# simzero/cudaParticlesFoam

Hardware: AMD Instinct MI355X
Metric: Mparticle-steps/s (higher is better)
Workload: dtype f64

## Files before the change

cudaparticlesfoam_amd/csrc/cpf_stream.hip:

```cpp
#include "cpf_stream_ops.h"

#include <hip/hip_ext.h>

#include <type_traits>

namespace cpf {

#ifndef CPF_STREAM_SLOTS
#define CPF_STREAM_SLOTS 6
#endif
#ifndef CPF_STREAM_SLOTS_FIXED
#define CPF_STREAM_SLOTS_FIXED 9
#endif
#ifndef CPF_STREAM_WAVES
#define CPF_STREAM_WAVES 7
#endif
constexpr int kSlotStride = 8;
#ifndef CPF_STREAM_GATHER_LANES
#define CPF_STREAM_GATHER_LANES 32
#endif
constexpr int kStreamGatherLanes = CPF_STREAM_GATHER_LANES;
#ifndef CPF_STREAM_PAIRED
#define CPF_STREAM_PAIRED 0
#endif
#ifndef CPF_STREAM_INROUND
#define CPF_STREAM_INROUND 0
#endif
#ifndef CPF_STREAM_HIT_POOL
#define CPF_STREAM_HIT_POOL 40
#endif
constexpr int kVertexTets = 12;
#ifndef CPF_VERTEX_BLOCKS
#define CPF_VERTEX_BLOCKS 4
#endif
#ifndef CPF_VERTEX_PICK_UNROLL
#define CPF_VERTEX_PICK_UNROLL 12
#endif
constexpr int kVertexBlocks = CPF_VERTEX_BLOCKS;
constexpr int kStreamSparsePerCell = 8;
constexpr int kSitOut = INT32_MIN + 7;

struct StreamKernArgs {
    double *x, *y, *z; int32_t* cell; const int64_t* gid; double* vel; int64_t n; double dt, sigma; uint32_t step0; int nCyc;
    uint32_t seed; MeshView m; unsigned long long* counters; StreamArgs sa;
};
static_assert(offsetof(StreamKernArgs, x) == 0 && offsetof(StreamKernArgs, cell) == 24, "kernarg_cloud_ptrs reads bytes 0..31");
constexpr int kKernArgHitSpill = (int)(offsetof(StreamKernArgs, sa) + offsetof(StreamArgs, hitSpill));
constexpr int kKernArgZBad = (int)(offsetof(StreamKernArgs, sa) + offsetof(StreamArgs, zBad));
constexpr int kKernArgGid = (int)offsetof(StreamKernArgs, gid), kKernArgSigma = (int)offsetof(StreamKernArgs, sigma);
constexpr int kKernArgStep0 = (int)offsetof(StreamKernArgs, step0), kKernArgSeed = (int)offsetof(StreamKernArgs, seed);
#ifndef CPF_STREAM_BROWN_KERNARG
#define CPF_STREAM_BROWN_KERNARG 1
#endif

#ifndef CPF_STREAM_L1_ZERO_SKIP
#define CPF_STREAM_L1_ZERO_SKIP 1
#endif
#ifndef CPF_STREAM_LAZY_USED
#define CPF_STREAM_LAZY_USED 1
#endif
#ifndef CPF_STREAM_BOX_SPARSE
#define CPF_STREAM_BOX_SPARSE 1
#endif
#ifndef CPF_STREAM_FLAT_KICK
#define CPF_STREAM_FLAT_KICK 0
#endif
#ifndef CPF_STREAM_FLAT_ZERO_SKIP
#define CPF_STREAM_FLAT_ZERO_SKIP 0
#endif
#ifndef CPF_STREAM_FLAT_Z
#define CPF_STREAM_FLAT_Z 1
#endif
#ifndef CPF_STREAM_SLOTS_BOX
#define CPF_STREAM_SLOTS_BOX 9
#endif
#ifndef CPF_STREAM_SLOTS_BOX_B
#define CPF_STREAM_SLOTS_BOX_B 12
#endif
#ifndef CPF_STREAM_WAVES_BOX_B
#define CPF_STREAM_WAVES_BOX_B 6
#endif
#ifndef CPF_STREAM_WAVES_BOX
#define CPF_STREAM_WAVES_BOX 6
#endif
#ifndef CPF_STREAM_WAVES_B1
#define CPF_STREAM_WAVES_B1 5
#endif
#ifndef CPF_STREAM_WAVES_L2
#define CPF_STREAM_WAVES_L2 6
#endif
#ifndef CPF_STREAM_WAVES_B0
#define CPF_STREAM_WAVES_B0 7
#endif
#ifndef CPF_STREAM_HIT_POOL_B0
#define CPF_STREAM_HIT_POOL_B0 18
#endif
#ifndef CPF_STREAM_WAVES_FLAT
#define CPF_STREAM_WAVES_FLAT CPF_STREAM_WAVES
#endif
#ifndef CPF_STREAM_WAVES_FLAT_BODY
#define CPF_STREAM_WAVES_FLAT_BODY 0
#endif
#ifndef CPF_FLAT_ROUND_GATHER
#define CPF_FLAT_ROUND_GATHER 1
#endif
#ifndef CPF_FLAT_ROUND_HINTS
#define CPF_FLAT_ROUND_HINTS 1
#endif
#ifndef CPF_FLAT_ROUND_ONE_HOOK
#define CPF_FLAT_ROUND_ONE_HOOK 1
#endif
#ifndef CPF_FLAT_ROUND_MASK
#define CPF_FLAT_ROUND_MASK 1
#endif
#ifndef CPF_FLAT_ROUND_OUTCOME
#define CPF_FLAT_ROUND_OUTCOME 1
#endif
#ifndef CPF_STREAM_SLOTS_BROWN
#define CPF_STREAM_SLOTS_BROWN 10
#endif
#ifndef CPF_STREAM_HIT_REGS_L2
#define CPF_STREAM_HIT_REGS_L2 0
#endif
#ifndef CPF_STREAM_WAVES_VERTEX
#define CPF_STREAM_WAVES_VERTEX 4
#endif
template <bool BROWNIAN, bool STORE_VEL, bool STATS, int LOOKUP>
struct StreamShape {
    static constexpr LookupMode mode = lookup_traits(LOOKUP);
    static_assert(mode.id == LOOKUP, "LOOKUP: a mode of kLookupModes");
    static constexpr int slots = [] {
        if (!mode.fixed) return CPF_STREAM_SLOTS;
        if (mode.box) return BROWNIAN ? CPF_STREAM_SLOTS_BOX_B : CPF_STREAM_SLOTS_BOX;
        if (BROWNIAN && LOOKUP == kLookupFixed) return CPF_STREAM_SLOTS_BROWN;
        return CPF_STREAM_SLOTS_FIXED;
    }();
    static_assert(slots >= 4 && slots <= 32, "slots");
    static constexpr int stride = mode.box ? 4 : kSlotStride;
    static constexpr bool hitInRegs = !BROWNIAN && (!mode.bigCells || CPF_STREAM_HIT_REGS_L2);
    static constexpr int pool = [] {
        if (hitInRegs) return 1;
        if (mode.mixed) return 16;
        if (BROWNIAN && LOOKUP == kLookupLoop) return CPF_STREAM_HIT_POOL_B0;
        return CPF_STREAM_HIT_POOL;
    }();
    static constexpr int waves = [] {
        if (STORE_VEL || STATS) return 1;
        if (mode.gatherAhead != 0) return BROWNIAN ? 4 : 5;
        if (BROWNIAN && mode.mixed) return 5;
        if (BROWNIAN && mode.box) return CPF_STREAM_WAVES_BOX_B;
        if (BROWNIAN) return LOOKUP == kLookupFixed ? CPF_STREAM_WAVES_B1 : CPF_STREAM_WAVES_B0;
        if (mode.bigCells) return CPF_STREAM_WAVES_L2;
        if (mode.box) return CPF_STREAM_WAVES_BOX;
        if (mode.mixed) return 6;
        if (LOOKUP == kLookupFlatLoop) return CPF_STREAM_WAVES_FLAT;
        return CPF_STREAM_WAVES;
    }();
};
#if CPF_STREAM_SLOTS == 6 && CPF_STREAM_SLOTS_FIXED == 9 && CPF_STREAM_SLOTS_BROWN == 10 && CPF_STREAM_SLOTS_BOX == 9 && CPF_STREAM_SLOTS_BOX_B == 12 && \
    CPF_STREAM_WAVES == 7 && CPF_STREAM_WAVES_B0 == 7 && CPF_STREAM_WAVES_B1 == 5 && CPF_STREAM_WAVES_L2 == 6 && CPF_STREAM_WAVES_BOX == 6 && \
    CPF_STREAM_WAVES_BOX_B == 6 && CPF_STREAM_WAVES_FLAT == 7 && CPF_STREAM_HIT_POOL == 40 && CPF_STREAM_HIT_POOL_B0 == 18 && CPF_STREAM_HIT_REGS_L2 == 0
template <int LOOKUP>
constexpr bool shape_is(int slots, int waves, int pool, int slotsB, int wavesB, int poolB) {
    using P = StreamShape<false, false, false, LOOKUP>; using B = StreamShape<true, false, false, LOOKUP>;
    return P::slots == slots && P::waves == waves && P::pool == pool && B::slots == slotsB && B::waves == wavesB && B::pool == poolB;
}
static_assert(shape_is<0>(6, 7, 1, 6, 7, 18) && shape_is<1>(9, 7, 1, 10, 5, 40) && shape_is<2>(9, 6, 16, 9, 5, 16) && shape_is<3>(9, 6, 1, 9, 5, 16) &&
              shape_is<4>(9, 5, 1, 9, 4, 40) && shape_is<5>(6, 6, 1, 6, 5, 16) && shape_is<6>(9, 6, 1, 12, 6, 40) && shape_is<8>(6, 7, 1, 6, 7, 40) &&
              shape_is<9>(9, 7, 1, 9, 7, 40) && shape_is<11>(9, 6, 1, 12, 5, 16), "StreamShape: slots, waves, pool per mode");
#endif

template <bool BROWNIAN, bool REFLECT, bool STORE_VEL, bool STATS, int LOOKUP, bool VERTEX, bool ZSET = false>
__device__ __forceinline__ void stream_body(
    const int64_t* __restrict__ gid, double* __restrict__ vel, int64_t n, double dt, double sigma, uint32_t step0,
    int nCyc, uint32_t seed, const MeshView& m, unsigned long long* __restrict__ counters, const StreamArgs& sa, const VertexField& vf) {
    using Shape = StreamShape<BROWNIAN, STORE_VEL, STATS, LOOKUP>;
    constexpr bool LOOKUP_FIXED = Shape::mode.fixed, mixed = Shape::mode.mixed, bigCells = Shape::mode.bigCells, BOX = Shape::mode.box;
    constexpr bool FLAT = Shape::mode.flat, HIT_IN_REGS = Shape::hitInRegs;
    constexpr int kGatherAhead = Shape::mode.gatherAhead, NS = Shape::slots, kStride = Shape::stride, kPool = Shape::pool;
    constexpr unsigned kRecBytes = 32u * kStride;
    constexpr unsigned ALL = NS == 32 ? 0xFFFFFFFFu : ((1u << NS) - 1u);
    __shared__ double4 slots[NS][kStride];
    __shared__ unsigned sCnt[4];
    constexpr bool kInRound = CPF_STREAM_INROUND == 2 || (CPF_STREAM_INROUND == 1 && BROWNIAN);
    static_assert(!(kInRound && mixed), "in-round reflection knows neither face groups nor two-record cells");
    static_assert(!ZSET || (FLAT && !BROWNIAN && !VERTEX), "settled z: the flat walk without the kick or the vertex advect");
    __shared__ double sLane[ZSET ? 2 : 3][64];
    __shared__ double sPool[3][kPool];
    __shared__ unsigned sPoolUsed;
    __shared__ double sPre[ZSET ? 160 : (BROWNIAN ? 288 : 224)];
    __shared__ double sCone[VERTEX ? kVertexBlocks : 1][VERTEX ? kVertexTets * 10 : 1];
    double(*sE)[64] = sLane;
    const int lane = threadIdx.x;
    const unsigned ul = threadIdx.x;
    const unsigned preBase = uniform32(lds_addr(sPre));
    const unsigned slotBase = uniform32(lds_addr(slots));
    const int tpc = sa.tilesPerChunk;
    constexpr bool kMaskBusy = ZSET && CPF_FLAT_ROUND_MASK != 0, kPlainOutcome = ZSET && CPF_FLAT_ROUND_OUTCOME != 0;
    constexpr bool kFlatGather = ZSET && CPF_FLAT_ROUND_GATHER != 0, kHints = ZSET && CPF_FLAT_ROUND_HINTS != 0;
    constexpr bool kOneHook = ZSET && CPF_FLAT_ROUND_ONE_HOOK != 0;
    const bool zKeep = ZSET || (FLAT && CPF_STREAM_FLAT_Z != 0 && sa.zSettled != 0);
    auto park = [&](const D3& e) __attribute__((always_inline)) {
        sE[0][lane] = e.x; sE[1][lane] = e.y;
        if (!ZSET) sE[2][lane] = e.z;
    };
    auto parked = [&]() __attribute__((always_inline)) -> D3 {
        if (ZSET) return {sE[0][lane], sE[1][lane], 0.0};
        return {sE[0][lane], sE[1][lane], sE[2][lane]};
    };
    const bool zFold = !BOX && BROWNIAN && REFLECT && m.zThin != 0;
    const bool zLast = !FLAT && !BROWNIAN && m.zPairLast != 0;
    const bool flatKick = zFold && m.zSide0 != 0;
    const unsigned nTiles = (unsigned)((n + 63) >> 6);
    const unsigned nFull = (unsigned)(n >> 6), nTail = (unsigned)n & 63u;
    const unsigned big = sa.bigChunks;
    const unsigned nChunks = big + (nTiles - big * (unsigned)tpc);
    auto chunk_first = [&](unsigned c) -> unsigned {
        return c < big ? c * (unsigned)tpc : big * (unsigned)tpc + (c - big);
    };
    auto chunk_tiles = [&](unsigned c, unsigned firstTile) -> int {
        if (c >= nChunks) return 0;
        const unsigned k = nTiles - firstTile;
        const unsigned want = c < big ? (unsigned)tpc : 1u;
        return (int)(k < want ? k : want);
    };
    auto chunk_of = [&](unsigned j) -> unsigned {
        const unsigned long long c = (unsigned long long)(blockIdx.x & (kStreamGroups - 1)) + (unsigned long long)kStreamGroups * j;
        return c < (unsigned long long)nChunks ? (unsigned)c : nChunks;
    };
    StepStats st = {0, 0, 0, 0};
#ifdef CPF_STREAM_TIMELINE
    const uint64_t tl0 = __builtin_amdgcn_s_memrealtime();
    unsigned tlTiles = 0, tlRounds = 0;
    unsigned tlWaitRec = 0, tlWaitEnd = 0, tlMissRounds = 0;
    unsigned long long* const tlH = (!STORE_VEL && vel != nullptr && (sa.debug & 4)) ? reinterpret_cast<unsigned long long*>(vel) + 8 * 16384 : nullptr;
    unsigned tlVis = 0, tlRoundIdx = 0;
#endif

    for (unsigned k = blockIdx.x; k < (unsigned)kStreamGroups; k += gridDim.x)
        if (lane == 0) sa.grabNext[k * kStreamCounterStride] = 0u;
    const unsigned grp = blockIdx.x & (kStreamGroups - 1);
    unsigned* const myGrab = sa.grab + grp * kStreamCounterStride;

    auto prefetch = [&](unsigned t, const CloudPtrs& cp) __attribute__((always_inline)) -> int {
        double* const x = cp.x; double* const y = cp.y; double* const z = cp.z; int32_t* const cell = cp.cell;
        t = uniform32(t);
        const int64_t b = (int64_t)t * 64;
        unsigned ul = threadIdx.x;
        asm volatile("" : "+v"(ul));
        if (t < nFull) {
            const char* s1 = (ul < 32u ? reinterpret_cast<const char*>(x + b) : reinterpret_cast<const char*>(y + b)) + (ul & 31u) * 16u;
            glds16(s1, preBase);
            if (zKeep) {
                if (ul < 16u) glds16(reinterpret_cast<const char*>(cell + b) + ul * 16u, preBase + 1024u);
            } else if (ul < 48u) {
                const char* s2 = ul < 32u ? reinterpret_cast<const char*>(z + b) + ul * 16u
                                          : reinterpret_cast<const char*>(cell + b) + (ul - 32u) * 16u;
                glds16(s2, preBase + 1024u);
            }
            if (BROWNIAN) {
                const int64_t* const g = CPF_STREAM_BROWN_KERNARG ? static_cast<const int64_t*>(kernarg_pointer<kKernArgGid>()) : gid;
                if (g != nullptr) {
                    if (ul < 32u) glds16(reinterpret_cast<const char*>(g + b) + ul * 16u, preBase + 1792u);
                    return 3;
                }
            }
            return 2;
        }
        const unsigned lim = nTail - 1u;
        const unsigned l = ul < lim ? ul : lim;
        if (zKeep) {
            const double vx = (x + b)[l], vy = (y + b)[l];
            const int vc = (cell + b)[l];
            sPre[ul] = vx; sPre[64 + ul] = vy;
            reinterpret_cast<int*>(sPre + 128)[ul] = vc;
        } else {
        const double vx = (x + b)[l], vy = (y + b)[l], vz = (z + b)[l];
        const int vc = (cell + b)[l];
        sPre[ul] = vx; sPre[64 + ul] = vy; sPre[128 + ul] = vz;
        reinterpret_cast<int*>(sPre + 192)[ul] = vc;
        }
        if (BROWNIAN) {
            const int64_t* const g = CPF_STREAM_BROWN_KERNARG ? static_cast<const int64_t*>(kernarg_pointer<kKernArgGid>()) : gid;
            if (g != nullptr) reinterpret_cast<int64_t*>(sPre + 224)[ul] = (g + b)[l];
        }
        return 0;
    };

    unsigned got0 = 0;
    if (lane == 0) got0 = grab_sync(myGrab);
    const unsigned chunk0 = chunk_of(uniform32(got0));
    if (chunk_tiles(chunk0, chunk_first(chunk0)) > 0) {
        int tagv = -1;
        unsigned fifo = 0;

        unsigned tile = chunk_first(chunk0);
        int tilesLeft = chunk_tiles(chunk0, tile);
        (void)prefetch(tile, kernarg_cloud_ptrs());
        wait_vmcnt<0>();

        bool havePrev = false;
        unsigned rtile = 0;
        double rvx = 0, rvy = 0, rvz = 0;
        bool ralive = false;
        int rc = 0;
        unsigned rlim = 63;

        for (;;) {
            tile = uniform32(tile);
            const unsigned plim = tile < nFull ? 63u : nTail - 1u;
            double px = sPre[ul], py = sPre[64 + ul], pz = 0.0;
            int pc;
            if (zKeep) pc = reinterpret_cast<const int*>(sPre + 128)[ul];
            else { pz = sPre[128 + ul]; pc = reinterpret_cast<const int*>(sPre + 192)[ul]; }
            uint64_t pid = 0;
            if (BROWNIAN) {
                const bool haveIds = (CPF_STREAM_BROWN_KERNARG ? kernarg_pointer<kKernArgGid>() : (void*)gid) != nullptr;
                pid = haveIds ? (uint64_t) reinterpret_cast<const int64_t*>(sPre + 224)[ul] : (uint64_t)tile * 64 + ul;
            }
            if (ul > plim || pc < 0) pc = CPF_CELL_FROZEN;
            if (FLAT && !ZSET && !zKeep && ballot64(pc >= 0 && !(fabs(pz) <= 1.7976931348623157e308)) != 0ull) {
                unsigned* const bad = static_cast<unsigned*>(kernarg_pointer<kKernArgZBad>());
                if (bad != nullptr && lane == 0) *bad = 1u;
            }

            int cur = pc;
            int key2 = 0, carNext = 0, carBest = -1;
            double carDT = 2.0;
            D3 S_ = {px, py, pz}, v = {0, 0, 0};
            const uint64_t id = pid;

            unsigned ntile = 0;
            int ntilesLeft = 0;

            auto hook = [&](const D3& prev) __attribute__((always_inline)) -> int {
                int younger = 0;
                __builtin_amdgcn_sched_barrier(0);
                if (tilesLeft > 1) {
                    ntile = tile + 1;
                    ntilesLeft = tilesLeft - 1;
                } else {
                    unsigned got = 0;
                    if (lane == 0) got = grab_sync(myGrab);
                    const unsigned nxt = chunk_of(uniform32(got));
                    ntile = chunk_first(nxt);
                    ntilesLeft = chunk_tiles(nxt, ntile);
                }
                const CloudPtrs cp = kernarg_cloud_ptrs();
                double* const x = cp.x; double* const y = cp.y; double* const z = cp.z; int32_t* const cell = cp.cell;
                if (havePrev && !(sa.debug & 1)) {
                    const int64_t b = (int64_t)uniform32(rtile) * 64;
                    if (STORE_VEL && ralive) {
                        double* vv = vel + 3 * b;
                        async_store(vv, ul * 24u, rvx); async_store(vv + 1, ul * 24u, rvy); async_store(vv + 2, ul * 24u, rvz);
                    }
                    if (ul <= rlim) {
                        async_store(x + b, ul * 8u, prev.x); async_store(y + b, ul * 8u, prev.y);
                        if (!zKeep) async_store(z + b, ul * 8u, prev.z);
                        async_store(cell + b, ul * 4u, rc);
                    }
                    younger += zKeep ? 3 : 4;
                }
                if (ntilesLeft > 0 && !(sa.debug & 2)) younger += prefetch(ntile, cp);
                __builtin_amdgcn_sched_barrier(0);
                return younger;
            };

            bool busy = false;
            unsigned long long busyM = 0ull;
            bool zUnclear = false;
            int token = INT32_MIN, h = 0, j = 0;
            int hitAt = -1;
            D3 hitReg = {0, 0, 0};
            auto park_hit = [&](const D3& Hp) __attribute__((always_inline)) {
                if (HIT_IN_REGS) { hitReg = Hp; return; }
                if (hitAt < 0) hitAt = (int)atomicAdd(&sPoolUsed, 1u);
                if (hitAt < kPool) { sPool[0][hitAt] = Hp.x; sPool[1][hitAt] = Hp.y; sPool[2][hitAt] = Hp.z; }
                else {
                    double* sp = static_cast<double*>(kernarg_pointer<kKernArgHitSpill>()) + (size_t)blockIdx.x * kStreamHitSpillDoubles;
                    async_store(sp, ul * 8u, Hp.x); async_store(sp + 64, ul * 8u, Hp.y); async_store(sp + 128, ul * 8u, Hp.z);
                }
            };

            auto cycle_begin = [&](int c) __attribute__((always_inline)) {
                if (cur < 0) cur = CPF_CELL_FROZEN;
                busy = cur >= 0;
                if (kMaskBusy) busyM = ballot64(cur >= 0);
                token = INT32_MIN; h = 0; j = 0;
                if (bigCells) key2 = 0;
                if (!HIT_IN_REGS && REFLECT) { hitAt = -1; if (lane == 0) sPoolUsed = 0u; }
                zUnclear = false;
                if (STATS && busy) ++st.steps;
                if (VERTEX) {
                    bool slow = busy;
#if defined(CPF_VERTEX_AB) && CPF_VERTEX_AB == 1
                    if (busy) { const double4 u = m.U[cur]; v = {u.x, u.y, u.z}; slow = false; }
#endif
                    if (vf.tetsPerCell == kVertexTets) {
                        unsigned long long todo = ballot64(slow);
                        while (todo != 0ull) {
                            int myBlock = -1;
                            __syncthreads();
#pragma unroll
                            for (int q = 0; q < kVertexBlocks; ++q) {
                                if (todo != 0ull) {
                                    const int ck = __builtin_amdgcn_readlane(cur, __ffsll((long long)todo) - 1);
                                    const bool mine = slow && cur == ck;
                                    if (mine) myBlock = q;
                                    if (lane < 5 * kVertexTets) {
                                        const int tk = lane / 5, piece = lane - 5 * tk;
                                        const double2 row = reinterpret_cast<const double2*>(vf.cone + kConeDoubles * ((int64_t)ck * kVertexTets + tk))[piece];
                                        reinterpret_cast<double2*>(&sCone[q][0] + 10 * tk)[piece] = row;
                                    }
                                    todo &= ~ballot64(mine);
                                }
                            }
                            __syncthreads();
                            if (myBlock >= 0) {
                                const double4 ap = vf.apex[cur];
                                const D3 A = {ap.x, ap.y, ap.z};
                                const D3 r = {S_.x - A.x, S_.y - A.y, S_.z - A.z};
                                int cand = 0;
                                double candMin = -1e300;
                                const double* blk = &sCone[myBlock][0];
#pragma unroll CPF_VERTEX_PICK_UNROLL
                                for (int k = 0; k < kVertexTets; ++k) {
                                    const double2* g = reinterpret_cast<const double2*>(blk + 10 * k);
                                    const double2 g01 = g[0], g23 = g[1], g45 = g[2], g67 = g[3], g89 = g[4];
                                    const double cb = fma(g23.x, r.z, fma(g01.y, r.y, g01.x * r.x)), cc = fma(g45.y, r.z, fma(g45.x, r.y, g23.y * r.x));
// ... 2 lines not shown
                                    if (mm > candMin) { candMin = mm; cand = k; }
                                }
#if defined(CPF_VERTEX_AB) && CPF_VERTEX_AB == 2
                                { const double4 u = m.U[cur]; v = {u.x + 1e-300 * cand, u.y, u.z}; slow = false; }
#else
                                D3 vv;
                                if (vertex_velocity_in_tet(vf, S_, A, (int64_t)cur * kVertexTets + cand, vv)) { v = vv; slow = false; }
#endif
                            }
                        }
                    }
                    if (slow) (void)vertex_velocity(vf, S_, cur, v);
                }
            };

            auto round = [&](bool hookDue, bool cycleStart, int c) __attribute__((always_inline)) {
#ifdef CPF_STREAM_TIMELINE
                ++tlRounds;
                bool tlSat = false;
#endif
                const unsigned long long busyMask = kMaskBusy ? busyM : ballot64(busy);
                if (kMaskBusy) busy = __builtin_amdgcn_inverse_ballot_w64(busyM);
                const D3 Epre = parked();
                const int lk = (bigCells && key2 != 0) ? key2 : cur;
                int myslot = -1;
                unsigned used = 0;
                unsigned long long missLanes = busyMask;
                if (LOOKUP_FIXED) {
                    const int cell0 = __builtin_amdgcn_readlane(lk, __ffsll((long long)busyMask) - 1);
                    const unsigned long long in0 = __builtin_amdgcn_uicmp((unsigned)lk, (unsigned)cell0, 32 ) & busyMask;
                    if (in0 == busyMask) {
                        const unsigned long long hitTag = __builtin_amdgcn_uicmp((unsigned)tagv, (unsigned)cell0, 32 ) & ALL;
                        if (hitTag != 0ull) {
                            myslot = __ffsll((long long)hitTag) - 1;
                            used = (unsigned)hitTag;
                            missLanes = 0ull;
                        }
                    } else {
#if CPF_STREAM_LAZY_USED
                        unsigned long long eqs[NS];
#pragma unroll
                        for (int k = 0; k < NS; ++k) {
                            const int tk = __builtin_amdgcn_readlane(tagv, k);
                            eqs[k] = __builtin_amdgcn_uicmp((unsigned)lk, (unsigned)tk, 32 );
                            asm("v_cndmask_b32_e64 %0, %1, %2, %3" : "=v"(myslot) : "v"(myslot), "n"(k), "s"(eqs[k]));
                        }
                        missLanes = ballot64(myslot < 0) & busyMask;
                        if (missLanes != 0ull) {
#pragma unroll
                            for (int k = 0; k < NS; ++k) used |= ((eqs[k] & busyMask) != 0ull ? 1u : 0u) << k;
                        }
#else
#pragma unroll
                        for (int k = 0; k < NS; ++k) {
                            const int tk = __builtin_amdgcn_readlane(tagv, k);
                            const unsigned long long eqK = __builtin_amdgcn_uicmp((unsigned)lk, (unsigned)tk, 32 );
                            const unsigned long long inK = eqK & busyMask;
                            asm("v_cndmask_b32_e64 %0, %1, %2, %3" : "=v"(myslot) : "v"(myslot), "n"(k), "s"(eqK));
                            used |= (inK != 0ull ? 1u : 0u) << k;
                            missLanes &= ~inK;
                        }
#endif
                    }
                } else {
                    unsigned long long todo = busyMask;
                    missLanes = 0ull;
                    while (todo != 0ull) {
                        const int leader = __ffsll((long long)todo) - 1;
                        const int ck = __builtin_amdgcn_readlane(lk, leader);
                        const bool mine = lk == ck;
                        const unsigned long long same = ballot64(mine) & busyMask;
                        const unsigned long long hitTag = __builtin_amdgcn_uicmp((unsigned)tagv, (unsigned)ck, 32 );
                        if (hitTag != 0ull) {
                            const int sl = __ffsll((long long)hitTag) - 1;
                            used |= 1u << sl;
                            if (mine) myslot = sl;
                        } else {
                            missLanes |= same;
                        }
                        todo &= ~same;
                    }
                }
                int nJobs = 0;
                if (missLanes != 0ull) {
#define CPF_JOB(J)                                                                                          \
                    if (missLanes != 0ull && used != ALL) {                                                 \
                        const int leader = __ffsll((long long)missLanes) - 1;                               \
                        const int ck = __builtin_amdgcn_readlane(lk, leader);                               \
                        const unsigned cand = ~used & ALL;                                                  \
                        const unsigned hi = cand & (ALL << fifo) & ALL;                                     \
                        const int victim = __ffs((int)(hi ? hi : cand)) - 1;                                \
                        fifo = (unsigned)(victim + 1) == (unsigned)NS ? 0u : (unsigned)(victim + 1);          \
                        used |= 1u << victim;                                                               \
                        if (lane == victim) tagv = ck;                                                      \
                        const bool mine = lk == ck;                                                         \
                        if (mine) myslot = victim;                                                          \
                        missLanes &= ~ballot64(mine);                                                       \
                        if (ul < kRecBytes / 16u)                                                            \
                            glds16(reinterpret_cast<const char*>(BOX ? m.boxRec : m.cellRec) + (int64_t)ck * kRecBytes + ul * 16u,  \
                                   uniform32(slotBase + (unsigned)victim * kRecBytes));                     \
                        nJobs = J + 1;                                                                      \
                    }
                    CPF_JOB(0) CPF_JOB(1) CPF_JOB(2) CPF_JOB(3)
                    if (LOOKUP_FIXED) { CPF_JOB(4) CPF_JOB(5) CPF_JOB(6) CPF_JOB(7) }
#undef CPF_JOB
                }
                int younger = 0;
                if (hookDue) younger = hook(Epre);
                if (BROWNIAN && cycleStart && busy) {
                    uint32_t kStep0 = step0, kSeed = seed;
                    if (CPF_STREAM_BROWN_KERNARG) kernarg_u32_pair<kKernArgStep0, kKernArgSeed>(kStep0, kSeed);
                    const D3 xi = normal3(id, kStep0 + (uint32_t)c, kSeed);
                    sE[0][lane] = xi.x; sE[1][lane] = xi.y; sE[2][lane] = xi.z;
                }
#ifdef CPF_STREAM_TIMELINE
                const uint64_t tlw0 = __builtin_amdgcn_s_memrealtime();
#endif
                if (nJobs != 0) {
                    if (ZSET) {
                        if (younger == 5) wait_vmcnt<5>();
                        else if (younger == 3) wait_vmcnt<3>();
                        else if (younger == 2) wait_vmcnt<2>();
                        else wait_vmcnt<0>();
                    } else
                    if (younger >= 7) wait_vmcnt<7>();
                    else if (younger == 6) wait_vmcnt<6>();
                    else if (younger == 5) wait_vmcnt<5>();
                    else if (younger >= 4) wait_vmcnt<4>();
                    else if (younger == 3) wait_vmcnt<3>();
                    else if (younger >= 2) wait_vmcnt<2>();
                    else wait_vmcnt<0>();
#ifdef CPF_STREAM_TIMELINE
                    tlWaitRec += (unsigned)(__builtin_amdgcn_s_memrealtime() - tlw0); ++tlMissRounds;
#endif
                }
                const bool gatherRound = __popcll(missLanes) >= kStreamGatherLanes;
                auto advect = [&](const double4* rec) __attribute__((always_inline)) -> D3 {
                    D3 Pn;
                    if (VERTEX) {
                        Pn = {S_.x + dt * v.x, S_.y + dt * v.y, S_.z + dt * v.z};
                    } else {
                        double4 u;
                        if (BOX) { const double2 uxy = reinterpret_cast<const double2*>(rec)[5]; u = {uxy.x, uxy.y, reinterpret_cast<const double*>(rec)[12], 0.0}; }
                        else u = rec[6];
                        v = {u.x, u.y, u.z};
                        if (ZSET) Pn = {fma(dt, v.x, S_.x), fma(dt, v.y, S_.y), 0.0};
                        else Pn = axpy(dt, v, S_);
                    }
                    D3 disp = {Pn.x - S_.x, Pn.y - S_.y, ZSET ? 0.0 : Pn.z - S_.z};
                    if (BROWNIAN) {
                        const D3 xi = {sE[0][lane], sE[1][lane], sE[2][lane]};
                        disp = axpy(CPF_STREAM_BROWN_KERNARG ? kernarg_f64<kKernArgSigma>() : sigma, xi, disp);
                    }
                    D3 E = {S_.x + disp.x, S_.y + disp.y, ZSET ? 0.0 : S_.z + disp.z};
                    if (BROWNIAN && REFLECT && zFold) {
                        bool clear;
                        const int nb = fold_z(E.z, S_.z, rec[BOX ? 0 : 4], rec[BOX ? 0 : 5], clear);
                        zUnclear |= ballot64(!clear) != 0ull;
                        if (STATS) st.refl += nb;
                        if (STORE_VEL && (nb & 1)) v.z = -v.z;
                    }
                    park(E);
                    return E;
                };
                if (busy) {
                    int next, outSlot = 0;
// ... 180 lines not shown
                    } else
                    do { round(hookDue, cycleStart, c); hookDue = false; cycleStart = false; } while (ballot64(busy) != 0ull);
#endif
#ifdef CPF_STREAM_TIMELINE
                    {
                        unsigned mx = tlVis;
                        for (int off = 32; off > 0; off >>= 1) { const unsigned o = (unsigned)__shfl_xor((int)mx, off, 64); mx = o > mx ? o : mx; }
                        const unsigned r = tlRoundIdx < 15u ? tlRoundIdx : 15u, iv = mx < 15u ? mx : 15u;
                        if (tlH != nullptr && lane == 0) atomicAdd(&tlH[16 * 65 + 16 + r * 16u + iv], 1ull);
                    }
#endif
                    if (live > 0) cycle_end();
#ifdef CPF_STREAM_CAP_TEST
                    if (capDropped) { S_ = capKeep; cur = capCur; }
#endif
                }
            } else {
                const D3 prev = parked();
                (void)hook(prev);
            }

#ifdef CPF_STREAM_TIMELINE
            const uint64_t tle0 = __builtin_amdgcn_s_memrealtime();
#endif
            wait_vmcnt<0>();
#ifdef CPF_STREAM_TIMELINE
            tlWaitEnd += (unsigned)(__builtin_amdgcn_s_memrealtime() - tle0);
            ++tlTiles;
#endif
            rtile = tile; havePrev = true;
            park(S_);
            if (STORE_VEL) { rvx = v.x; rvy = v.y; rvz = v.z; ralive = pc >= 0; }
            rc = cur;
            rlim = plim;
            if (ntilesLeft <= 0) break;
            tile = ntile; tilesLeft = ntilesLeft;
        }
        {
            const int64_t b = (int64_t)rtile * 64;
            const CloudPtrs cp = kernarg_cloud_ptrs();
            double* const x = cp.x; double* const y = cp.y; double* const z = cp.z; int32_t* const cell = cp.cell;
            const D3 res = parked();
            if (ul <= rlim) {
                (x + b)[ul] = res.x; (y + b)[ul] = res.y;
                if (!zKeep) (z + b)[ul] = res.z;
                (cell + b)[ul] = rc;
            }
            if (STORE_VEL && ralive) {
                double* vv = vel + 3 * b;
                vv[3 * ul] = rvx; vv[3 * ul + 1] = rvy; vv[3 * ul + 2] = rvz;
            }
        }
    }
#ifdef CPF_STREAM_TIMELINE
    if (!STORE_VEL && vel != nullptr && lane == 0) {
        uint64_t* o = reinterpret_cast<uint64_t*>(vel) + 8 * (uint64_t)blockIdx.x;
        o[0] = tl0; o[1] = __builtin_amdgcn_s_memrealtime(); o[2] = tlTiles; o[3] = tlRounds;
        o[4] = tlWaitRec; o[5] = tlWaitEnd; o[6] = tlMissRounds; o[7] = 0;
    }
#endif
    if (STATS) flush_stats(st, counters, sCnt);
}

template <bool BROWNIAN, bool REFLECT, bool STORE_VEL, bool STATS, int LOOKUP>
__global__ __launch_bounds__(64, (StreamShape<BROWNIAN, STORE_VEL, STATS, LOOKUP>::waves)) void step_kernel_stream(
    double* __restrict__ , double* __restrict__ , double* __restrict__ , int32_t* __restrict__ ,
    const int64_t* __restrict__ gid, double* __restrict__ vel, int64_t n, double dt, double sigma, uint32_t step0,
    int nCyc, uint32_t seed, MeshView m, unsigned long long* __restrict__ counters, StreamArgs sa) {
    stream_body<BROWNIAN, REFLECT, STORE_VEL, STATS, LOOKUP, false>(gid, vel, n, dt, sigma, step0, nCyc, seed, m, counters, sa, VertexField{});
}

template <bool BROWNIAN, bool REFLECT, bool STORE_VEL, bool STATS, int LOOKUP>
__global__ __launch_bounds__(64, ((STORE_VEL || STATS) ? 1 : CPF_STREAM_WAVES_VERTEX)) void step_kernel_stream_vertex(
    double* __restrict__ , double* __restrict__ , double* __restrict__ , int32_t* __restrict__ ,
    const int64_t* __restrict__ gid, double* __restrict__ vel, int64_t n, double dt, double sigma, uint32_t step0,
    int nCyc, uint32_t seed, MeshView m, unsigned long long* __restrict__ counters, StreamArgs sa, VertexField vf) {
    stream_body<BROWNIAN, REFLECT, STORE_VEL, STATS, LOOKUP, true>(gid, vel, n, dt, sigma, step0, nCyc, seed, m, counters, sa, vf);
}

template <bool REFLECT, bool STORE_VEL, bool STATS, int LOOKUP>
__global__ __launch_bounds__(64, (StreamShape<false, STORE_VEL, STATS, LOOKUP>::waves)) void step_kernel_stream_flat(
    double* __restrict__ , double* __restrict__ , double* __restrict__ , int32_t* __restrict__ ,
    const int64_t* __restrict__ gid, double* __restrict__ vel, int64_t n, double dt, double sigma, uint32_t step0,
    int nCyc, uint32_t seed, MeshView m, unsigned long long* __restrict__ counters, StreamArgs sa) {
    stream_body<false, REFLECT, STORE_VEL, STATS, LOOKUP, false, true>(gid, vel, n, dt, sigma, step0, nCyc, seed, m, counters, sa, VertexField{});
}

template <bool B, bool R_, bool SV, bool ST, int LF, bool VX = false, bool ZS = false>
static hipError_t launch_stream_inst(hipStream_t st, double* x, double* y, double* z, int32_t* cell, const int64_t* gid,
                                     double* vel, int64_t n, double dt, double sigma, uint32_t step0, int nCyc,
                                     uint32_t seed, const MeshView& m, unsigned long long* counters, StreamState& ss,
                                     const VertexField* vf, bool settled, hipEvent_t evStart, hipEvent_t evStop) {
    constexpr LookupMode mode = lookup_traits(LF);
    constexpr auto kernel = [] {
        if constexpr (VX) return &step_kernel_stream_vertex<B, R_, SV, ST, LF>;
        else if constexpr (ZS) return &step_kernel_stream_flat<R_, SV, ST, LF>;
        else return &step_kernel_stream<B, R_, SV, ST, LF>;
    }();
    static int wavesPerCU = 0;
    if (wavesPerCU == 0) {
        int nb = 0;
        const hipError_t e = hipOccupancyMaxActiveBlocksPerMultiprocessor(&nb, kernel, 64, 0);
        if (e != hipSuccess) return e;
        wavesPerCU = nb < 1 ? 1 : (nb > 32 ? 32 : nb);
        if (ZS && CPF_STREAM_WAVES_FLAT_BODY > 0 && wavesPerCU > 4 * CPF_STREAM_WAVES_FLAT_BODY) wavesPerCU = 4 * CPF_STREAM_WAVES_FLAT_BODY;
    }
    const int64_t nTiles = (n + 63) >> 6;
    if (nTiles >= ((int64_t)1 << 31)) return hipErrorInvalidValue;
    const int64_t slotsOnChip = (int64_t)((ss.wavesPerCU > 0 && !VX) ? ss.wavesPerCU : wavesPerCU) * ss.numCU;
    int tpc = ss.tilesPerChunk > 0 ? ss.tilesPerChunk : (!mode.fixed ? 4 : 3);
    const double tailFraction = ss.tailFraction >= 0.0 ? ss.tailFraction : (!mode.fixed ? 0.1 : 0.2);
    while (tpc > 1 && nTiles / tpc < 4 * slotsOnChip) tpc = tpc > 2 ? tpc - 1 : 1;
    int64_t bigChunks = (int64_t)((double)(nTiles / tpc) * (1.0 - tailFraction));
    if (tpc == 1 || bigChunks < 0) bigChunks = 0;
    const int64_t nChunks = bigChunks + (nTiles - bigChunks * tpc);
    int64_t R = slotsOnChip / kStreamGroups;
    const int64_t need = (nChunks + kStreamGroups - 1) / kStreamGroups;
    if (R > need) R = need;
    if (R < 1) R = 1;
    unsigned* cur = ss.d_grab + (size_t)(ss.parity & 1) * kStreamGroups * kStreamCounterStride;
    unsigned* nxt = ss.d_grab + (size_t)((ss.parity & 1) ^ 1) * kStreamGroups * kStreamCounterStride;
    if (R * kStreamGroups > ss.hitSpillWaves) R = ss.hitSpillWaves / kStreamGroups;
    if (R < 1 || ss.d_hitSpill == nullptr) return hipErrorInvalidValue;
    const bool zSettled = mode.flat && !VX && settled && ss.flatZ != 0;
    if (ZS != zSettled && mode.flat && !VX) return hipErrorInvalidValue;
    StreamArgs sa = {cur, nxt, (int)R, tpc, (unsigned)bigChunks, ss.debug, ss.d_hitSpill, zSettled ? 1 : 0, ss.zBad};
    auto launch = [&](const auto&... tail) {
        const dim3 grid((unsigned)(R * kStreamGroups));
        if (evStart != nullptr && evStop != nullptr)
            hipExtLaunchKernelGGL(kernel, grid, dim3(64), 0, st, evStart, evStop, 0, x, y, z, cell, gid, vel, n, dt, sigma, step0, nCyc,
                                  seed, m, counters, sa, tail...);
        else
            hipLaunchKernelGGL(kernel, grid, dim3(64), 0, st, x, y, z, cell, gid, vel, n, dt, sigma, step0, nCyc, seed, m, counters, sa,
                               tail...);
        return stream_launch_done(st, ss);
    };
    if constexpr (VX) return vf == nullptr ? hipErrorInvalidValue : launch(*vf);
    else return launch();
}

static int stream_lookup_mode(int64_t n, const MeshView& m, const StreamState& ss, bool brown, bool vertex) {
    int64_t cells = m.nCells;
    if (ss.densityLookup && ss.occupiedHost != nullptr) {
        const int64_t occ = (int64_t)ss.occupiedHost[0], live = (int64_t)ss.occupiedHost[1];
        if (occ > 0 && occ <= cells && live > 0 && live <= 2 * n && n <= 2 * live) cells = occ;
    }
    if (vertex) {
        if (ss.lookup == kLookupLoop || ss.lookup == kLookupFixed) return ss.lookup;
        return n < 128 * cells ? kLookupFixed : kLookupLoop;
    }
    if (m.mixed == 1 && m.boxRec != nullptr && m.zThin == 0 && ss.lookup < 0) return kLookupBoxGroups;
    if (m.mixed == 2) return kLookupMixedBig;
    if (m.mixed) return (ss.lookup >= 0 ? ss.lookup == kLookupLoop : n >= 128 * cells) ? kLookupMixedLoop : kLookupMixed;
    const bool box = m.boxRec != nullptr && m.zThin == 0;
    if (ss.lookup >= 0) return (ss.lookup == kLookupBox && !box) ? kLookupFixed : ss.lookup;
    if (box && CPF_STREAM_BOX_SPARSE) return kLookupBox;
    if (n < kStreamSparsePerCell * cells) return kLookupSparse;
    const bool flat = !brown && ss.flat && ss.flatField && m.zSide0 != 0;
    if (n < 128 * cells) return flat ? kLookupFlatFixed : kLookupFixed;
    return flat ? kLookupFlatLoop : kLookupLoop;
}

StepPlan plan_step(const MeshView& m, const StreamState& ss, int variant, const VertexField* vf, int64_t n, int nCyc, double D,
                   unsigned flags, bool stats) {
    StepPlan p;
    p.brown = D > 0.0;
    p.reflect = (flags & CPF_STEP_NO_REFLECT) == 0;
    p.storeVel = (flags & CPF_STEP_STORE_VEL) != 0;
    p.stats = stats;
    const int coopMaxCells = (ss.coopMaxCells <= 0 || ss.coopMaxCells > kCoopMaxCells) ? kCoopMaxCells : ss.coopMaxCells;
    if (!m.allHex) {
        const bool wantsStream = variant == kVariantAuto || variant == kVariantStream || variant == kVariantCoop;
        variant = (m.mixed && m.cellRec && wantsStream) ? kVariantStream : kVariantGeneric;
    } else {
        if (variant == kVariantAuto)
            variant = !(nCyc >= kFusedCoopCycles && m.nCells <= coopMaxCells) ? kVariantStream : kVariantCoop;
        if (variant == kVariantCoop && m.nCells > coopMaxCells) variant = kVariantStream;
#ifndef CPF_EXPERIMENTS
        if (variant == kVariantFixed || variant == kVariantFixedScalar) variant = kVariantCoop;
        if (variant == kVariantAhead) variant = kVariantStream;
#endif
    }
    if (vf != nullptr) {
        p.cone = vf->cone != nullptr;
        const bool streams = p.cone && vf->tetsPerCell == 12 && m.mixed == 0 && m.cellRec != nullptr && variant == kVariantStream;
        p.kernel = streams ? StepPlan::kStreamVertex : StepPlan::kVertex;
        if (streams) p.lookup = stream_lookup_mode(n, m, ss, p.brown, true);
        return p;
    }
    if (variant == kVariantAhead && (p.brown || p.storeVel || nCyc != 1)) variant = kVariantStream;
    p.kernel = (StepPlan::Kernel)variant;
    if (variant == kVariantStream) p.lookup = stream_lookup_mode(n, m, ss, p.brown, false);
    return p;
}

constexpr bool vertex_mode(LookupMode r) { return !(r.mixed || r.box || r.flat || r.gatherAhead != 0); }
hipError_t launch_step_stream(const StepPlan& p, hipStream_t st, double* x, double* y, double* z, int32_t* cell, const int64_t* gid,
                              double* vel, int64_t n, double dt, double sigma, uint32_t step0, int nCyc, uint32_t seed,
                              const MeshView& m, unsigned long long* counters, const VertexField* vf, StreamState& ss, bool zSettled,
                              hipEvent_t evStart, hipEvent_t evStop) {
    return with_bools([&](auto B, auto R, auto SV, auto ST) {
        auto inst = [&](auto kick, auto LF, auto VX, auto ZS) {
            return launch_stream_inst<kick, R, SV, ST, LF, VX, ZS>(st, x, y, z, cell, gid, vel, n, dt, sigma, step0, nCyc, seed, m, counters,
                                                                   ss, vf, zSettled, evStart, evStop);
        };
        constexpr std::true_type yes{}; constexpr std::false_type no{};
        if (p.kernel == StepPlan::kStreamVertex)
            return with_lookup(p.lookup, [&](auto LF) {
                if constexpr (vertex_mode(lookup_traits(LF))) return inst(B, LF, yes, no);
                else return hipErrorInvalidValue;
            });
        const bool body = p.flat_body(ss, zSettled);
        return with_lookup(p.lookup, [&](auto LF) {
            if constexpr (!lookup_traits(LF).flat) return inst(B, LF, no, no);
            else if constexpr (B) return hipErrorInvalidValue;
            else return body ? inst(no, LF, no, yes) : inst(no, LF, no, no);
        });
    }, p.brown, p.reflect, p.storeVel, p.stats);
}

// ... 2 lines not shown
```

cudaparticlesfoam_amd/csrc/cpf_stream_ops.h:

```cpp
#pragma once
#include "cpf_walk.h"

namespace cpf {

#ifndef CPF_STREAM_GROUPS
#define CPF_STREAM_GROUPS 256
#endif
constexpr int kStreamGroups = CPF_STREAM_GROUPS;
constexpr int kStreamCounterStride = 16;

typedef __attribute__((address_space(3))) const char* lds_cptr;
__device__ __forceinline__ unsigned lds_addr(const void* p) {
    return (unsigned)(uintptr_t)(lds_cptr)p;
}
__device__ __forceinline__ unsigned uniform32(unsigned v) { return (unsigned)__builtin_amdgcn_readfirstlane((int)v); }
__device__ __forceinline__ int64_t uniform64(int64_t v) {
    const unsigned lo = uniform32((unsigned)v), hi = uniform32((unsigned)((uint64_t)v >> 32));
    return (int64_t)(((uint64_t)hi << 32) | lo);
}
__device__ __forceinline__ void glds16(const void* gsrc, unsigned ldsDst) {
    unsigned keep;
    asm volatile("s_waitcnt lgkmcnt(0)\n\ts_mov_b32 %0, m0\n\ts_mov_b32 m0, %2\n\ts_nop 0\n\t"
                 "global_load_lds_dwordx4 %1, off\n\ts_mov_b32 m0, %0"
                 : "=&s"(keep) : "v"(gsrc), "s"(ldsDst) : "memory");
}
__device__ __forceinline__ void async_store(double* base, unsigned byteOff, double v) {
    asm volatile("s_nop 4\n\tglobal_store_dwordx2 %0, %1, %2" : : "v"(byteOff), "v"(v), "s"(base) : "memory");
}
__device__ __forceinline__ void async_store(int32_t* base, unsigned byteOff, int v) {
    asm volatile("s_nop 4\n\tglobal_store_dword %0, %1, %2" : : "v"(byteOff), "v"(v), "s"(base) : "memory");
}
__device__ __forceinline__ unsigned grab_sync(unsigned* base) {
    unsigned r;
    asm volatile("s_nop 4\n\tglobal_atomic_add %0, %1, %2, %3 sc0\n\ts_waitcnt vmcnt(0)" : "=&v"(r) : "v"(0u), "v"(1u), "s"(base) : "memory");
    return r;
}
__device__ __forceinline__ void load3_sync(const double* base, unsigned byteOff, double& a, double& b, double& c) {
    asm volatile("s_waitcnt vmcnt(0)\n\ts_nop 4\n\tglobal_load_dwordx2 %0, %3, %4 sc0 sc1\n\tglobal_load_dwordx2 %1, %3, %4 offset:512 sc0 sc1\n\t"
                 "global_load_dwordx2 %2, %3, %4 offset:1024 sc0 sc1\n\ts_waitcnt vmcnt(0)"
                 : "=&v"(a), "=&v"(b), "=&v"(c) : "v"(byteOff), "s"(base) : "memory");
}
struct CloudPtrs { double* x; double* y; double* z; int32_t* cell; };
__device__ __forceinline__ CloudPtrs kernarg_cloud_ptrs() {
    typedef unsigned u32x8 __attribute__((ext_vector_type(8)));
    u32x8 r;
    asm volatile("s_load_dwordx8 %0, %1, 0x0\n\ts_waitcnt lgkmcnt(0)" : "=s"(r) : "s"(__builtin_amdgcn_kernarg_segment_ptr()) : "memory");
    auto ptr = [](unsigned lo, unsigned hi) { return (uintptr_t)(((unsigned long long)hi << 32) | lo); };
    return {reinterpret_cast<double*>(ptr(r[0], r[1])), reinterpret_cast<double*>(ptr(r[2], r[3])),
            reinterpret_cast<double*>(ptr(r[4], r[5])), reinterpret_cast<int32_t*>(ptr(r[6], r[7]))};
}
template <int BYTE_OFFSET>
__device__ __forceinline__ void* kernarg_pointer() {
    typedef unsigned u32x2 __attribute__((ext_vector_type(2)));
    u32x2 r;
    asm volatile("s_load_dwordx2 %0, %1, %2\n\ts_waitcnt lgkmcnt(0)" : "=s"(r) : "s"(__builtin_amdgcn_kernarg_segment_ptr()), "n"(BYTE_OFFSET) : "memory");
    return reinterpret_cast<void*>((uintptr_t)(((unsigned long long)r[1] << 32) | r[0]));
}
template <int OFF_A, int OFF_B>
__device__ __forceinline__ void kernarg_u32_pair(uint32_t& a, uint32_t& b) {
    asm volatile("s_load_dword %0, %2, %3\n\ts_load_dword %1, %2, %4\n\ts_waitcnt lgkmcnt(0)"
                 : "=&s"(a), "=&s"(b) : "s"(__builtin_amdgcn_kernarg_segment_ptr()), "n"(OFF_A), "n"(OFF_B) : "memory");
}
template <int BYTE_OFFSET>
__device__ __forceinline__ double kernarg_f64() {
    typedef unsigned u32x2 __attribute__((ext_vector_type(2)));
    u32x2 r;
    asm volatile("s_load_dwordx2 %0, %1, %2\n\ts_waitcnt lgkmcnt(0)" : "=s"(r) : "s"(__builtin_amdgcn_kernarg_segment_ptr()), "n"(BYTE_OFFSET) : "memory");
    return __longlong_as_double((long long)(((unsigned long long)r[1] << 32) | r[0]));
}
template <int N>
__device__ __forceinline__ void wait_vmcnt() { asm volatile("s_waitcnt vmcnt(%0)" : : "n"(N) : "memory"); }

struct StreamArgs {
    unsigned* grab;
    unsigned* grabNext;
    int wavesPerGroup;
    int tilesPerChunk;
    unsigned bigChunks;
    int debug;
    double* hitSpill;
    int zSettled;
    unsigned* zBad;
};

inline hipError_t stream_launch_done(hipStream_t st, StreamState& ss) {
    const hipError_t e = hipGetLastError();
    if (e == hipSuccess) { ss.parity ^= 1; return e; }
    (void)hipMemsetAsync(ss.d_grab, 0, kStreamGrabBytes, st);
    return e;
}

}
```

Before: 109,000.

## Deal flat-walk chunks from a shrinking multi-level table passed in kernargs

Replaces the two-level big/tail chunk scheme for the settled-z flat stream kernel with a four-level deal table whose chunk sizes shrink (8, 4, 2, then 1 tile by default). The table is passed as an extra kernel argument and read with scalar loads. The aim is better load balance at the tail of the dynamic work grab, while keeping large chunks early to amortise grab atomics. It also adds a leaner loop form of the per-round cell-record miss job allocation. In exchange, each grab now costs a few extra scalar kernarg loads, and the plan logic on the host is more complex.

```diff
diff --git a/cudaparticlesfoam_amd/csrc/cpf_deal.h b/cudaparticlesfoam_amd/csrc/cpf_deal.h
--- /dev/null
+++ b/cudaparticlesfoam_amd/csrc/cpf_deal.h
@@ -0,0 +1,106 @@
+#pragma once
+#include <cstdint>
+
+#if defined(__HIPCC__)
+#define CPF_DEAL_HD __host__ __device__ __attribute__((always_inline))
+#else
+#define CPF_DEAL_HD
+#endif
+
+namespace cpf {
+
+constexpr int kDealLevels = 4;
+struct DealRow { unsigned firstChunk, firstTile, tiles, aux; };
+struct DealPlan {
+    unsigned bound[kDealLevels];
+    DealRow row[kDealLevels];
+    unsigned& own_first() { return row[0].aux; }
+    unsigned own_first() const { return row[0].aux; }
+};
+static_assert(sizeof(DealPlan) == 16 + 16 * kDealLevels, "DealPlan: the kernel reads it from the kernarg segment in 16-byte pieces");
+
+#ifndef CPF_FLAT_DEAL_TILES
+#define CPF_FLAT_DEAL_TILES 8
+#endif
+#ifndef CPF_FLAT_DEAL_SHARE0
+#define CPF_FLAT_DEAL_SHARE0 40
+#endif
+#ifndef CPF_FLAT_DEAL_SHARE1
+#define CPF_FLAT_DEAL_SHARE1 30
+#endif
+#ifndef CPF_FLAT_DEAL_SHARE2
+#define CPF_FLAT_DEAL_SHARE2 20
+#endif
+#ifndef CPF_FLAT_DEAL_MIN_CHUNKS
+#define CPF_FLAT_DEAL_MIN_CHUNKS 4
+#endif
+static_assert(CPF_FLAT_DEAL_TILES >= 1 && CPF_FLAT_DEAL_TILES <= 1024 && CPF_FLAT_DEAL_SHARE0 >= 0 && CPF_FLAT_DEAL_SHARE1 >= 0 &&
+              CPF_FLAT_DEAL_SHARE2 >= 0 && CPF_FLAT_DEAL_SHARE0 + CPF_FLAT_DEAL_SHARE1 + CPF_FLAT_DEAL_SHARE2 <= 100, "dealing knobs");
+
+CPF_DEAL_HD inline unsigned deal_level(unsigned c, unsigned b0, unsigned b1, unsigned b2) {
+    return c < b0 ? 0u : (c < b1 ? 1u : (c < b2 ? 2u : 3u));
+}
+CPF_DEAL_HD inline unsigned deal_chunk(unsigned c, unsigned nChunks, unsigned nTiles, const DealRow& r, unsigned& first) {
+    first = r.firstTile + (c - r.firstChunk) * r.tiles;
+    if (c >= nChunks || first >= nTiles) return 0u;
+    const unsigned k = nTiles - first;
+    return k < r.tiles ? k : r.tiles;
+}
+
+inline DealPlan deal_plan_from(int64_t nTiles, const int64_t (*levels)[2], int count) {
+    DealPlan p{};
+    int64_t chunk = 0, tile = 0;
+    int l = 0;
+    for (; l < count && l < kDealLevels - 1; ++l) {
+        int64_t tiles = levels[l][1] < 1 ? 1 : levels[l][1], chunks = levels[l][0] < 0 ? 0 : levels[l][0];
+        if (chunks > (nTiles - tile) / tiles) chunks = (nTiles - tile) / tiles;
+        p.row[l] = {(unsigned)chunk, (unsigned)tile, (unsigned)tiles, 0u};
+        chunk += chunks; tile += chunks * tiles;
+        p.bound[l] = (unsigned)chunk;
+    }
+    for (; l < kDealLevels; ++l) {
+        p.row[l] = {(unsigned)chunk, (unsigned)tile, 1u, 0u};
+        chunk += nTiles - tile; tile = nTiles;
+        p.bound[l] = (unsigned)chunk;
+    }
+    return p;
+}
+inline int64_t deal_chunks(const DealPlan& p) { return (int64_t)p.bound[kDealLevels - 1]; }
+
+inline int64_t deal_two_level(int64_t nTiles, int64_t slotsOnChip, double tailFraction, int& tpc) {
+    while (tpc > 1 && nTiles / tpc < 4 * slotsOnChip) tpc = tpc > 2 ? tpc - 1 : 1;
+    int64_t bigChunks = (int64_t)((double)(nTiles / tpc) * (1.0 - tailFraction));
+    if (tpc == 1 || bigChunks < 0) bigChunks = 0;
+    return bigChunks;
+}
+inline DealPlan deal_plan_two_level(int64_t nTiles, int64_t slotsOnChip, double tailFraction, int tpc) {
+    const int64_t big = deal_two_level(nTiles, slotsOnChip, tailFraction, tpc);
+    const int64_t levels[1][2] = {{big, tpc}};
+    return deal_plan_from(nTiles, levels, 1);
+}
+inline DealPlan deal_plan_shrinking(int64_t nTiles, int64_t slotsOnChip, int first = CPF_FLAT_DEAL_TILES) {
+    const int share[3] = {CPF_FLAT_DEAL_SHARE0, CPF_FLAT_DEAL_SHARE1, CPF_FLAT_DEAL_SHARE2};
+    for (int t = first < 1 ? 1 : first;; t /= 2) {
+        int64_t levels[3][2];
+        for (int l = 0; l < 3; ++l) {
+            const int64_t tiles = (t >> l) > 1 ? (t >> l) : 1;
+            levels[l][0] = nTiles * share[l] / 100 / tiles;
+            levels[l][1] = tiles;
+        }
+        const DealPlan p = deal_plan_from(nTiles, levels, 3);
+        if (t <= 1 || deal_chunks(p) >= CPF_FLAT_DEAL_MIN_CHUNKS * slotsOnChip) return p;
+    }
+}
+
+inline int deal_plan_check(const DealPlan& p, int64_t nTiles) {
+    int64_t chunk = 0, tile = 0;
+    for (int l = 0; l < kDealLevels; ++l) {
+        if (p.row[l].firstChunk != chunk || p.row[l].firstTile != tile) return 1;
+        if (p.row[l].tiles < 1 || p.bound[l] < p.row[l].firstChunk) return 2;
+        tile += (int64_t)(p.bound[l] - p.row[l].firstChunk) * p.row[l].tiles;
+        chunk = p.bound[l];
+    }
+    return tile == nTiles ? 0 : 3;
+}
+
+}
diff --git a/cudaparticlesfoam_amd/csrc/cpf_stream.hip b/cudaparticlesfoam_amd/csrc/cpf_stream.hip
--- a/cudaparticlesfoam_amd/csrc/cpf_stream.hip
+++ b/cudaparticlesfoam_amd/csrc/cpf_stream.hip
@@ -47,6 +47,10 @@
 static_assert(offsetof(StreamKernArgs, x) == 0 && offsetof(StreamKernArgs, cell) == 24, "kernarg_cloud_ptrs reads bytes 0..31");
 constexpr int kKernArgHitSpill = (int)(offsetof(StreamKernArgs, sa) + offsetof(StreamArgs, hitSpill));
 constexpr int kKernArgZBad = (int)(offsetof(StreamKernArgs, sa) + offsetof(StreamArgs, zBad));
+struct FlatKernArgs { StreamKernArgs a; DealPlan deal; };
+constexpr int kKernArgDealBounds = (int)(offsetof(FlatKernArgs, deal) + offsetof(DealPlan, bound));
+constexpr int kKernArgDealRows = (int)(offsetof(FlatKernArgs, deal) + offsetof(DealPlan, row));
+static_assert(offsetof(FlatKernArgs, deal) == sizeof(StreamKernArgs) && sizeof(DealRow) == 16, "the table follows StreamArgs without a gap");
 constexpr int kKernArgGid = (int)offsetof(StreamKernArgs, gid), kKernArgSigma = (int)offsetof(StreamKernArgs, sigma);
 constexpr int kKernArgStep0 = (int)offsetof(StreamKernArgs, step0), kKernArgSeed = (int)offsetof(StreamKernArgs, seed);
 #ifndef CPF_STREAM_BROWN_KERNARG
@@ -100,6 +104,18 @@
 #endif
 #ifndef CPF_STREAM_WAVES_FLAT_BODY
 #define CPF_STREAM_WAVES_FLAT_BODY 0
+#endif
+#ifndef CPF_FLAT_DEAL_TABLE
+#define CPF_FLAT_DEAL_TABLE 1
+#endif
+#ifndef CPF_FLAT_JOB_LEAN
+#define CPF_FLAT_JOB_LEAN 1
+#endif
+#ifndef CPF_FLAT_JOB_LOOP
+#define CPF_FLAT_JOB_LOOP 0
+#endif
+#ifndef CPF_FLAT_DEAL_OWN_FIRST
+#define CPF_FLAT_DEAL_OWN_FIRST 0
 #endif
 #ifndef CPF_FLAT_ROUND_GATHER
 #define CPF_FLAT_ROUND_GATHER 1
@@ -199,6 +215,7 @@
     constexpr bool kMaskBusy = ZSET && CPF_FLAT_ROUND_MASK != 0, kPlainOutcome = ZSET && CPF_FLAT_ROUND_OUTCOME != 0;
     constexpr bool kFlatGather = ZSET && CPF_FLAT_ROUND_GATHER != 0, kHints = ZSET && CPF_FLAT_ROUND_HINTS != 0;
     constexpr bool kOneHook = ZSET && CPF_FLAT_ROUND_ONE_HOOK != 0;
+    constexpr bool kLeanJob = ZSET && CPF_FLAT_JOB_LEAN != 0;
     const bool zKeep = ZSET || (FLAT && CPF_STREAM_FLAT_Z != 0 && sa.zSettled != 0);
     auto park = [&](const D3& e) __attribute__((always_inline)) {
         sE[0][lane] = e.x; sE[1][lane] = e.y;
@@ -228,6 +245,14 @@
         const unsigned long long c = (unsigned long long)(blockIdx.x & (kStreamGroups - 1)) + (unsigned long long)kStreamGroups * j;
         return c < (unsigned long long)nChunks ? (unsigned)c : nChunks;
     };
+    constexpr bool kDealTable = ZSET && CPF_FLAT_DEAL_TABLE != 0;
+    auto deal = [&](unsigned j, unsigned& first) __attribute__((always_inline)) -> int {
+        const kernarg_u32x4 b = kernarg_u32_quad<kKernArgDealBounds>();
+        const unsigned long long c64 = (unsigned long long)(blockIdx.x & (kStreamGroups - 1)) + (unsigned long long)kStreamGroups * j;
+        const unsigned c = c64 < (unsigned long long)b[3] ? (unsigned)c64 : b[3];
+        const kernarg_u32x4 r = kernarg_u32_quad_at(uniform32((unsigned)kKernArgDealRows + 16u * deal_level(c, b[0], b[1], b[2])));
+        return (int)deal_chunk(c, b[3], nTiles, DealRow{r[0], r[1], r[2], 0u}, first);
+    };
     StepStats st = {0, 0, 0, 0};
 #ifdef CPF_STREAM_TIMELINE
     const uint64_t tl0 = __builtin_amdgcn_s_memrealtime();
@@ -288,14 +313,20 @@
     };
 
     unsigned got0 = 0;
+    unsigned ownFirst = 0;
+    if (kDealTable && CPF_FLAT_DEAL_OWN_FIRST != 0) ownFirst = kernarg_u32_quad<kKernArgDealRows>()[3];
+    if (kDealTable && CPF_FLAT_DEAL_OWN_FIRST != 0 && ownFirst != 0u) got0 = blockIdx.x / (unsigned)kStreamGroups;
+    else
     if (lane == 0) got0 = grab_sync(myGrab);
-    const unsigned chunk0 = chunk_of(uniform32(got0));
-    if (chunk_tiles(chunk0, chunk_first(chunk0)) > 0) {
+    const unsigned chunk0 = kDealTable ? 0u : chunk_of(uniform32(got0));
+    unsigned tile0 = 0;
+    const int tiles0 = kDealTable ? deal(uniform32(got0), tile0) : 0;
+    if (kDealTable ? tiles0 > 0 : chunk_tiles(chunk0, chunk_first(chunk0)) > 0) {
         int tagv = -1;
         unsigned fifo = 0;
 
-        unsigned tile = chunk_first(chunk0);
-        int tilesLeft = chunk_tiles(chunk0, tile);
+        unsigned tile = kDealTable ? tile0 : chunk_first(chunk0);
+        int tilesLeft = kDealTable ? tiles0 : chunk_tiles(chunk0, tile);
         (void)prefetch(tile, kernarg_cloud_ptrs());
         wait_vmcnt<0>();
 
@@ -342,9 +373,12 @@
                 } else {
                     unsigned got = 0;
                     if (lane == 0) got = grab_sync(myGrab);
+                    if (kDealTable) ntilesLeft = deal(ownFirst + uniform32(got), ntile);
+                    else {
                     const unsigned nxt = chunk_of(uniform32(got));
                     ntile = chunk_first(nxt);
                     ntilesLeft = chunk_tiles(nxt, ntile);
+                    }
                 }
                 const CloudPtrs cp = kernarg_cloud_ptrs();
                 double* const x = cp.x; double* const y = cp.y; double* const z = cp.z; int32_t* const cell = cp.cell;
@@ -513,6 +547,34 @@
                     }
                 }
                 int nJobs = 0;
+                if (kLeanJob) {
+                    if (missLanes != 0ull) {
+                        unsigned freeM = ~used & ALL;
+#if CPF_FLAT_JOB_LOOP
+#pragma nounroll
+#else
+#pragma unroll
+#endif
+                        for (int J = 0; J < (LOOKUP_FIXED ? 8 : 4); ++J) {
+                            if (freeM == 0u) break;
+                            const int leader = __builtin_ctzll(missLanes);
+                            const int ck = __builtin_amdgcn_readlane(lk, leader);
+                            const unsigned hi = freeM & (ALL << fifo);
+                            const int victim = __builtin_ctz(hi ? hi : freeM);
+                            fifo = (unsigned)(victim + 1) == (unsigned)NS ? 0u : (unsigned)(victim + 1);
+                            freeM &= ~(1u << victim);
+                            if (lane == victim) tagv = ck;
+                            const bool mine = lk == ck;
+                            if (mine) myslot = victim;
+                            missLanes &= ~ballot64(mine);
+                            if (ul < kRecBytes / 16u)
+                                glds16(reinterpret_cast<const char*>(m.cellRec) + (int64_t)ck * kRecBytes + ul * 16u,
+                                       uniform32(slotBase + (unsigned)victim * kRecBytes));
+                            nJobs = J + 1;
+                            if (missLanes == 0ull) break;
+                        }
+                    }
+                } else
                 if (missLanes != 0ull) {
 #define CPF_JOB(J)                                                                                          \
                     if (missLanes != 0ull && used != ALL) {                                                 \
@@ -859,7 +921,7 @@
 __global__ __launch_bounds__(64, (StreamShape<false, STORE_VEL, STATS, LOOKUP>::waves)) void step_kernel_stream_flat(
     double* __restrict__ , double* __restrict__ , double* __restrict__ , int32_t* __restrict__ ,
     const int64_t* __restrict__ gid, double* __restrict__ vel, int64_t n, double dt, double sigma, uint32_t step0,
-    int nCyc, uint32_t seed, MeshView m, unsigned long long* __restrict__ counters, StreamArgs sa) {
+    int nCyc, uint32_t seed, MeshView m, unsigned long long* __restrict__ counters, StreamArgs sa, DealPlan ) {
     stream_body<false, REFLECT, STORE_VEL, STATS, LOOKUP, false, true>(gid, vel, n, dt, sigma, step0, nCyc, seed, m, counters, sa, VertexField{});
 }
 
@@ -887,10 +949,17 @@
     const int64_t slotsOnChip = (int64_t)((ss.wavesPerCU > 0 && !VX) ? ss.wavesPerCU : wavesPerCU) * ss.numCU;
     int tpc = ss.tilesPerChunk > 0 ? ss.tilesPerChunk : (!mode.fixed ? 4 : 3);
     const double tailFraction = ss.tailFraction >= 0.0 ? ss.tailFraction : (!mode.fixed ? 0.1 : 0.2);
-    while (tpc > 1 && nTiles / tpc < 4 * slotsOnChip) tpc = tpc > 2 ? tpc - 1 : 1;
-    int64_t bigChunks = (int64_t)((double)(nTiles / tpc) * (1.0 - tailFraction));
-    if (tpc == 1 || bigChunks < 0) bigChunks = 0;
-    const int64_t nChunks = bigChunks + (nTiles - bigChunks * tpc);
+    const int tpcAsked = tpc;
+    const int64_t bigChunks = deal_two_level(nTiles, slotsOnChip, tailFraction, tpc);
+    int64_t nChunks = bigChunks + (nTiles - bigChunks * tpc);
+    DealPlan plan{};
+    if (ZS) {
+        const bool pinned = ss.tilesPerChunk > 0 || ss.tailFraction >= 0.0;
+        plan = (CPF_FLAT_DEAL_TABLE != 0 && !pinned && !mode.fixed) ? deal_plan_shrinking(nTiles, slotsOnChip)
+                                                                    : deal_plan_two_level(nTiles, slotsOnChip, tailFraction, tpcAsked);
+        if (deal_plan_check(plan, nTiles) != 0) return hipErrorInvalidValue;
+        if (CPF_FLAT_DEAL_TABLE != 0) nChunks = deal_chunks(plan);
+    }
     int64_t R = slotsOnChip / kStreamGroups;
     const int64_t need = (nChunks + kStreamGroups - 1) / kStreamGroups;
     if (R > need) R = need;
@@ -912,7 +981,9 @@
                                tail...);
         return stream_launch_done(st, ss);
     };
+    if (ZS && CPF_FLAT_DEAL_TABLE != 0 && CPF_FLAT_DEAL_OWN_FIRST != 0 && ss.wavesPerCU == 0) plan.own_first() = (unsigned)R;
     if constexpr (VX) return vf == nullptr ? hipErrorInvalidValue : launch(*vf);
+    else if constexpr (ZS) return launch(plan);
     else return launch();
 }
 
diff --git a/cudaparticlesfoam_amd/csrc/cpf_stream_ops.h b/cudaparticlesfoam_amd/csrc/cpf_stream_ops.h
--- a/cudaparticlesfoam_amd/csrc/cpf_stream_ops.h
+++ b/cudaparticlesfoam_amd/csrc/cpf_stream_ops.h
@@ -1,4 +1,5 @@
 #pragma once
+#include "cpf_deal.h"
 #include "cpf_walk.h"
 
 namespace cpf {
@@ -68,6 +69,18 @@
     asm volatile("s_load_dwordx2 %0, %1, %2\n\ts_waitcnt lgkmcnt(0)" : "=s"(r) : "s"(__builtin_amdgcn_kernarg_segment_ptr()), "n"(BYTE_OFFSET) : "memory");
     return __longlong_as_double((long long)(((unsigned long long)r[1] << 32) | r[0]));
 }
+typedef unsigned kernarg_u32x4 __attribute__((ext_vector_type(4)));
+template <int BYTE_OFFSET>
+__device__ __forceinline__ kernarg_u32x4 kernarg_u32_quad() {
+    kernarg_u32x4 r;
+    asm volatile("s_load_dwordx4 %0, %1, %2\n\ts_waitcnt lgkmcnt(0)" : "=s"(r) : "s"(__builtin_amdgcn_kernarg_segment_ptr()), "n"(BYTE_OFFSET) : "memory");
+    return r;
+}
+__device__ __forceinline__ kernarg_u32x4 kernarg_u32_quad_at(unsigned byteOffset) {
+    kernarg_u32x4 r;
+    asm volatile("s_load_dwordx4 %0, %1, %2\n\ts_waitcnt lgkmcnt(0)" : "=s"(r) : "s"(__builtin_amdgcn_kernarg_segment_ptr()), "s"(byteOffset) : "memory");
+    return r;
+}
 template <int N>
 __device__ __forceinline__ void wait_vmcnt() { asm volatile("s_waitcnt vmcnt(%0)" : : "n"(N) : "memory"); }
 
```

After: 105,200. 0.965x the previous value.
